# JingruiYu/FishBirdEyeVisualSLAM

Hardware: AMD Instinct MI355X
Metric: frames/s (extract+match+pose-opt), 1280x720+512x512 pair (higher is better)
Workload: dtype u8 (extract, Hamming) + f64 (pose optimisation); 1 GPU; configs[2]: 1280x720 front + 512x512 bird pair, HIP ORB extract + M3/M9 Hamming match + PoseOptimizationWithBird (~2k front + ~1k bird edges); nfeatures=2000, parallelism=replicas x1

## Files before the change

fishbirdeyevisualslam_amd/csrc/orb.hip:

```cpp
#include "fb_common.h"
#include "fb_fast_score.h"
#include "fb_primitives.h"

namespace {

constexpr int EDGE_THRESHOLD = 19;
constexpr int HALF_PATCH = 15;
constexpr int PATCH_SIZE = 31;
constexpr int BORDER = EDGE_THRESHOLD - 3;

constexpr int PATTERN_XY[1024] = {
#include "orb_pattern.inc"
};
constexpr int pattern_extreme(bool wantMax) {
  int m = PATTERN_XY[0];
  for (int i = 1; i < 1024; i++) m = wantMax ? (PATTERN_XY[i] > m ? PATTERN_XY[i] : m) : (PATTERN_XY[i] < m ? PATTERN_XY[i] : m);
  return m;
}
constexpr int PAT_BIAS = -pattern_extreme(false);
static_assert(PAT_BIAS >= 0 && pattern_extreme(true) + PAT_BIAS <= 255, "a pattern coordinate does not fit a biased byte");
struct PackedPattern { uint32_t test[256]; };
constexpr PackedPattern pack_pattern() {
  PackedPattern p{};
  for (int t = 0; t < 256; t++)
    for (int k = 0; k < 4; k++) p.test[t] |= (uint32_t)(PATTERN_XY[t * 4 + k] + PAT_BIAS) << (8 * k);
  return p;
}
__constant__ PackedPattern c_pattern = pack_pattern();

struct LevelInfo {
  int w, h, pitch;
  long long off;
  int nCols, nRows, wCell, hCell, cellBase;
  int N;
  long long candBase;
  int candCap;
  int slotCap;
  int outBase, outCap;
  int nIni;
  float hX;
  float scale;
  int patchSize;
  long long boff;
};

struct OrbK {
  int nlevels, iniTh, minTh, totalCells, outStride, capOut;
  int kpStride;
  int fastTileBytes, fastMaxOut, fastMaxPix;
  int fastTP;
  int dbg;
  unsigned long long *timers;
  int cellBase[FB_MAX_LEVELS + 1];
  int grpBase[FB_MAX_LEVELS + 1];
  int totalGroups;
  int descBase[FB_MAX_LEVELS + 1];
  int runBase[FB_MAX_LEVELS];
  int runCap[FB_MAX_LEVELS];
  long long pyrStride;
  long long blurStride;
  int blurStrips[FB_MAX_LEVELS + 1];
  long long candStride;
  int umax[16];
  LevelInfo L[FB_MAX_LEVELS];
};

struct ResizeTabs {
  const int *xofs;
  const short *ialpha;
  const int *yofs;
  const short *ibeta;
};

__device__ __forceinline__ int win_byte(uint32_t w0, uint32_t w1, uint32_t w2, uint32_t w3, int k) {
  const uint32_t lo = k & 8 ? w2 : w0, hi = k & 8 ? w3 : w1;
  const uint32_t w = k & 4 ? hi : lo;
  return (w >> (8 * (k & 3))) & 0xFF;
}

__global__ __launch_bounds__(256) void k_resize(const uint8_t *__restrict__ src0, long long srcImgStride, int sw,
                                                int sh, int spitch, uint8_t *__restrict__ dst0, long long dstImgStride,
                                                int dw, int dh, int dpitch, ResizeTabs tb) {
// ... 792 lines not shown
        const int r0 = min(tid * perj, J), r1 = min(r0 + perj, J);
        for (int r = r0; r < r1; r++) {
          const int p = order[r];
          for (int q = 0; q < 4; q++)
            if (ccnt[4 * p + q] > 0) {
              const int pos = totalKids - 1 - ci++;
              cpos[4 * p + q] = (unsigned short)pos;
              nxt[pos] = child_of(cur[p], q, ccnt[4 * p + q]);
            }
        }
        for (int p = a0; p < a1; p++)
          if (!split[p]) { npos[p] = (unsigned short)kp; nxt[kp++] = cur[p]; }
      }
    }
    const int Snew = totalKids + totalKeep;
    __syncthreads();
    for (int k0 = tid; k0 < n; k0 += NT * 4) {
      int pk[4];
      uint32_t ck[4];
#pragma unroll
      for (int u = 0; u < 4; u++) { const int kk = min(k0 + u * NT, n - 1); pk[u] = nof[kk]; ck[u] = cd[kk]; }
#pragma unroll
      for (int u = 0; u < 4; u++) {
        const int k = k0 + u * NT;
        if (k >= n) break;
        const int p = pk[u];
        if (split[p]) {
          const uint32_t c = ck[u];
          nof[k] = cpos[4 * p + quadrant(cur[p], (int)(c & 0xFFF) - BORDER, (int)((c >> 12) & 0xFFF) - BORDER)];
        } else nof[k] = npos[p];
      }
    }
    int myExp = 0;
    {
      const int pern = (Snew + NT - 1) / NT;
      const int n0 = min(tid * pern, Snew), n1 = min(n0 + pern, Snew);
      for (int p = n0; p < n1; p++) myExp += (p < totalKids && nxt[p].cnt > 1);
    }
    int nToExpand;
    fb::block_excl_scan<NT>(myExp, s_w, &nToExpand);
    if (tid == 0) s_nexp = nToExpand;
    __syncthreads();
    ONode *t = cur; cur = nxt; nxt = t;
    S = Snew;
    if (S >= N || S == prevSize) break;
    if (!finalPhase) {
      if (S + nToExpand * 3 > N) finalPhase = true;
    }
  }
  for (int p = tid; p < S; p += NT) best[p] = 0ull;
  __syncthreads();
  for (int k0 = tid; k0 < n; k0 += NT * 4) {
    int pk[4];
    uint32_t ck[4];
#pragma unroll
    for (int u = 0; u < 4; u++) { const int kk = min(k0 + u * NT, n - 1); pk[u] = nof[kk]; ck[u] = cd[kk]; }
#pragma unroll
    for (int u = 0; u < 4; u++) {
    const int k = k0 + u * NT;
    if (k >= n) break;
    const uint32_t c = ck[u];
    const int x = c & 0xFFF, y = (c >> 12) & 0xFFF, r = c >> 24;
    const int cellI = (y - EDGE_THRESHOLD) / Lv.hCell, cellJ = (x - EDGE_THRESHOLD) / Lv.wCell;
    const int dwid = min(Lv.wCell, Lv.w - 2 * EDGE_THRESHOLD - cellJ * Lv.wCell);
    const int inCell = (y - EDGE_THRESHOLD - cellI * Lv.hCell) * dwid + (x - EDGE_THRESHOLD - cellJ * Lv.wCell);
    const unsigned orderKey = (unsigned)(cellI * Lv.nCols + cellJ) * 4096u + (unsigned)inCell;
    const unsigned long long key = ((unsigned long long)r << 56) | ((unsigned long long)(0xFFFFFFFFu - orderKey) << 24) | (unsigned)k;
    atomicMax(&best[pk[u]], key);
    }
  }
  __syncthreads();
  for (int p = tid; p < S; p += NT) out[p] = cd[(unsigned)(best[p] & 0xFFFFFFull)];
  if (tid == 0) *outCount = S;
}

constexpr int BLUR_ROWS = 32;

__device__ __forceinline__ int reflect101(int i, int n) {
  if (i < 0) i = -i;
  if (i >= n) i = 2 * n - 2 - i;
  return i;
}

__global__ __launch_bounds__(256) void k_blur(OrbK K, const uint8_t *__restrict__ img0, long long imgStride, int pitch0,
                                              const uint8_t *__restrict__ pyr, uint8_t *__restrict__ blur) {
  const int b = blockIdx.y;
  const int strip = __builtin_amdgcn_readfirstlane(blockIdx.x * 4 + (threadIdx.x >> 6));
  const int lane = threadIdx.x & 63;
  if (strip >= K.blurStrips[K.nlevels]) return;
  int l = 0;
  while (strip >= K.blurStrips[l + 1]) l++;
  const LevelInfo &L = K.L[l];
  const int w = L.w, h = L.h;
  const int sidx = strip - K.blurStrips[l];
  const int nsx = (w + 255) >> 8;
  const int sy = sidx / nsx, sx = sidx - sy * nsx;
  const int x0 = sx * 256 + lane * 4;
  const int y0 = sy * BLUR_ROWS;
  if (x0 >= w) return;
  const uint8_t *img;
  int pitch;
  if (l == 0) { img = img0 + (long long)b * imgStride; pitch = pitch0; }
  else { img = pyr + (long long)b * K.pyrStride + L.off; pitch = L.pitch; }
  uint8_t *out = blur + (long long)b * K.blurStride + L.boff;
  const bool edge = x0 < 4 || x0 + 8 > w;
  const int base = edge ? max(min(x0 - 4, w - 12), 0) : x0 - 4;
  uint32_t m1[3] = {0, 0, 0}, m2[3] = {0, 0, 0};
  if (edge) {
#pragma unroll
    for (int i = 0; i < 12; i++) {
      const int c = reflect101(min(x0 - 4 + i, w + 2), w);
      const int sidx8 = min(max(c - base, 0), 11);
      const uint32_t lo = sidx8 < 8 ? (uint32_t)sidx8 : 0x0cu, hi = sidx8 < 8 ? 0x0cu : (uint32_t)(sidx8 - 8);
      m1[i >> 2] |= lo << (8 * (i & 3));
      m2[i >> 2] |= hi << (8 * (i & 3));
    }
  }
  const bool anyEdge = __ballot(edge) != 0ull;
  const uint32_t WA = 18u | (34u << 8) | (49u << 16) | (55u << 24), WB = 49u | (34u << 8) | (18u << 16);
  uint32_t pairs[6][4];
  uint32_t prevh[4] = {0u, 0u, 0u, 0u};
  constexpr int BLUR_PF = 4;
  uint32_t q[BLUR_PF][3];
  auto loadRow = [&](int r, uint32_t (&dst)[3]) {
    const int ys = reflect101(min(y0 + r - 3, h + 2), h);
    const uint8_t *row = img + (uint32_t)__mul24(ys, pitch);
    const uint32_t *pw = reinterpret_cast<const uint32_t *>(row + base);
    dst[0] = pw[0]; dst[1] = pw[1]; dst[2] = pw[2];
  };
#pragma unroll
  for (int r = 0; r < BLUR_PF; r++) loadRow(r, q[r]);
#pragma unroll
  for (int r = 0; r < BLUR_ROWS + 6; r++) {
    const int yo = y0 + r - 6;
    if (r >= 6 && yo >= h) break;
    uint32_t w0 = q[r % BLUR_PF][0], w1 = q[r % BLUR_PF][1], w2 = q[r % BLUR_PF][2];
    if (r + BLUR_PF < BLUR_ROWS + 6) loadRow(r + BLUR_PF, q[r % BLUR_PF]);
    if (anyEdge) {
      const uint32_t e0 = __builtin_amdgcn_perm(w1, w0, m1[0]) | __builtin_amdgcn_perm(w2, w2, m2[0]);
      const uint32_t e1 = __builtin_amdgcn_perm(w1, w0, m1[1]) | __builtin_amdgcn_perm(w2, w2, m2[1]);
      const uint32_t e2 = __builtin_amdgcn_perm(w1, w0, m1[2]) | __builtin_amdgcn_perm(w2, w2, m2[2]);
      if (edge) { w0 = e0; w1 = e1; w2 = e2; }
    }
    uint32_t hr[4];
    hr[0] = __builtin_amdgcn_udot4(__builtin_amdgcn_alignbyte(w2, w1, 1), WB, __builtin_amdgcn_udot4(__builtin_amdgcn_alignbyte(w1, w0, 1), WA, 0u, false), false);
    hr[1] = __builtin_amdgcn_udot4(__builtin_amdgcn_alignbyte(w2, w1, 2), WB, __builtin_amdgcn_udot4(__builtin_amdgcn_alignbyte(w1, w0, 2), WA, 0u, false), false);
    hr[2] = __builtin_amdgcn_udot4(__builtin_amdgcn_alignbyte(w2, w1, 3), WB, __builtin_amdgcn_udot4(__builtin_amdgcn_alignbyte(w1, w0, 3), WA, 0u, false), false);
    hr[3] = __builtin_amdgcn_udot4(w2, WB, __builtin_amdgcn_udot4(w1, WA, 0u, false), false);
    if (r >= 6) {
      typedef unsigned short u16x2b __attribute__((ext_vector_type(2)));
      const u16x2b W01 = {18, 34}, W23 = {49, 55}, W45 = {49, 34};
      uint32_t packed = 0;
#pragma unroll
      for (int k = 0; k < 4; k++) {
        uint32_t sum = (uint32_t)__mul24(18, (int)hr[k]) + (1u << 15);
        sum = __builtin_amdgcn_udot2(__builtin_bit_cast(u16x2b, pairs[(r + 1) % 6][k]), W01, sum, false);
        sum = __builtin_amdgcn_udot2(__builtin_bit_cast(u16x2b, pairs[(r + 3) % 6][k]), W23, sum, false);
        sum = __builtin_amdgcn_udot2(__builtin_bit_cast(u16x2b, pairs[(r + 5) % 6][k]), W45, sum, false);
        packed |= (uint32_t)min((int)(sum >> 16), 255) << (8 * k);
      }
      *reinterpret_cast<uint32_t *>(out + (uint32_t)(__mul24(yo, L.pitch) + x0)) = packed;
    }
#pragma unroll
    for (int k = 0; k < 4; k++) { pairs[r % 6][k] = prevh[k] | (hr[k] << 16); prevh[k] = hr[k]; }
  }
}

constexpr int DP_RAW_DW = 9, DP_RAW_ROWS = 31;
constexpr int DP_BL_DW = 10, DP_BL_ROWS = 37;

constexpr int DESC_WPB = 4;
constexpr int DESC_KPW = 2;

__global__ __launch_bounds__(64 * DESC_WPB) __attribute__((amdgpu_waves_per_eu(5, 5)))
void k_describe(OrbK K, const uint8_t *__restrict__ img0, long long imgStride,
                                                 int pitch0, const uint8_t *__restrict__ pyr,
                                                 const uint8_t *__restrict__ blur, const uint4 *__restrict__ angTab,
                                                 const uint32_t *__restrict__ lvlOut, const int *__restrict__ lvlCount,
                                                 fb_keypoint *__restrict__ kps, uint8_t *__restrict__ desc,
                                                 int32_t *__restrict__ nOut) {
  __shared__ __attribute__((aligned(16))) uint32_t rawp_all[DESC_WPB][DP_RAW_ROWS * DP_RAW_DW + 4];
  __shared__ __attribute__((aligned(16))) uint32_t blp_all[DESC_WPB][DP_BL_ROWS * DP_BL_DW + 2];
  const int b = blockIdx.y, lane = threadIdx.x & 63;
  const int wv = __builtin_amdgcn_readfirstlane(threadIdx.x >> 6);
  uint32_t *rawp = rawp_all[wv], *blp = blp_all[wv];
  const uint4 pq = reinterpret_cast<const uint4 *>(c_pattern.test)[lane];
  const uint4 angT = angTab[lane < 62 ? lane : 0];
  const int wg = (int)(blockIdx.x & 7) * (int)(gridDim.x >> 3) + (int)(blockIdx.x >> 3);
  int l = 0, runBase = K.runBase[0], runCap = K.runCap[0];
#pragma unroll
  for (int i = 1; i < FB_MAX_LEVELS; i++)
    if (i < K.nlevels && wg >= K.descBase[i]) { l = i; runBase = K.runBase[i]; runCap = K.runCap[i]; }
  const int slot = ((wg - K.descBase[l]) * DESC_WPB + wv) * DESC_KPW;
  const uint32_t *run = lvlOut + (long long)b * K.outStride + runBase;
  uint32_t rec[DESC_KPW];
#pragma unroll
  for (int j = 0; j < DESC_KPW; j++) rec[j] = run[min(slot + j, runCap - 1)];
  const int *cnts = lvlCount + b * K.nlevels;
  int below = 0, total = 0, mine = 0;
#pragma unroll
  for (int i = 0; i < FB_MAX_LEVELS; i++) {
    const int ci = cnts[i];
    const int c = i < K.nlevels ? ci : 0;
    total += c; below += i < l ? c : 0; mine = i == l ? c : mine;
  }
  const LevelInfo &Lv = K.L[l];
  const int lvPitch = Lv.pitch, lvPatch = Lv.patchSize;
  const long long lvOff = Lv.off, lvBoff = Lv.boff;
  const float lvScale = Lv.scale;
  const int nk = min(total, K.capOut);
  if (wg == 0 && threadIdx.x == 0) nOut[b] = nk;
  const int first = below + slot;
  const int nmine = min(DESC_KPW, min(mine - slot, nk - first));
  if (K.dbg == 11) { if ((int)(pq.x + pq.w) + (int)angT.x + (int)rec[0] + (int)rec[DESC_KPW - 1] + nmine + lvPitch + lvPatch + (int)lvOff + (int)lvBoff + (int)lvScale == 1234567) nOut[0] = 1; return; }
  if (nmine <= 0) return;
  const uint4 angW = make_uint4(angT.x & 0x0f0f0f0fu, angT.y & 0x0f0f0f0fu, angT.z & 0x0f0f0f0fu, angT.w & 0x0f0f0f0fu);
  const uint4 angK = make_uint4((angT.x >> 4) & 0x01010101u, (angT.y >> 4) & 0x01010101u, (angT.z >> 4) & 0x01010101u, (angT.w >> 4) & 0x01010101u);
  const uint8_t *lvImg = l == 0 ? img0 + (long long)b * imgStride : pyr + (long long)b * K.pyrStride + lvOff;
  const int rawPitch = l == 0 ? pitch0 : lvPitch;
  const uint8_t *lvBlur = blur + (long long)b * K.blurStride + lvBoff;
  const bool rawAligned = ((reinterpret_cast<uintptr_t>(lvImg) | (uintptr_t)rawPitch) & 3) == 0;
  constexpr int NB_IT = (DP_BL_ROWS + 5) / 6, NR_IT = (DP_RAW_ROWS + 6) / 7;
  const int rb0 = (lane * 205) >> 11, dwb = lane - rb0 * DP_BL_DW;
  const int rr0 = (lane * 57) >> 9, dwr = lane - rr0 * DP_RAW_DW;
  struct KP {
    int cx, cy, resp, pitch, bpitch, bxa, box, rxa, rox;
    const uint8_t *img, *bbase;
    bool rawAligned;
  };
  auto decode = [&](int j) {
    KP k;
    const uint32_t r = rec[j];
    k.cx = r & 0xFFF; k.cy = (r >> 12) & 0xFFF; k.resp = r >> 24;
    k.img = lvImg; k.pitch = rawPitch; k.bbase = lvBlur; k.bpitch = lvPitch; k.rawAligned = rawAligned;
    k.bxa = (k.cx - 18) & ~3; k.box = (k.cx - 18) - k.bxa;
    k.rxa = (k.cx - 15) & ~3;
    k.rox = k.rawAligned ? (k.cx - 15) - k.rxa : 0;
    return k;
  };
  uint32_t vb[DESC_KPW][NB_IT], vr[DESC_KPW][NR_IT];
  auto issue = [&](const KP &k, uint32_t (&vb)[NB_IT], uint32_t (&vr)[NR_IT]) {
    {
      uint32_t off = (uint32_t)(__mul24(k.cy - 18 + rb0, k.bpitch) + k.bxa + min(dwb, DP_BL_DW - 1) * 4);
// ... 27 lines not shown
      for (int i = lane; i < DP_RAW_ROWS * 31; i += 64) {
        const int yy = i / 31, xx = i - yy * 31;
        rb[yy * (DP_RAW_DW * 4) + xx] = k.img[(long long)(k.cy - 15 + yy) * k.pitch + k.cx - 15 + xx];
      }
    }
    __builtin_amdgcn_fence(__ATOMIC_RELEASE, "wavefront");
    __builtin_amdgcn_wave_barrier();
    __builtin_amdgcn_fence(__ATOMIC_ACQUIRE, "wavefront");
  };
  KP kpv[DESC_KPW];
#pragma unroll
  for (int j = 0; j < DESC_KPW; j++) {
    kpv[j] = decode(j);
    if (j < nmine) issue(kpv[j], vb[j], vr[j]);
  }
#pragma unroll
  for (int j = 0; j < DESC_KPW; j++) {
    if (j >= nmine) break;
    const KP &cur = kpv[j];
    stage(cur, vb[j], vr[j]);
    int m10 = 0, m01 = 0;
    if (lane < 62) {
      const int r = lane >> 1, half = lane & 1;
      const int sb = cur.rox + (half ? 15 : 0);
      const uint32_t *rowd = rawp + r * DP_RAW_DW + (sb >> 2);
      const uint32_t sh = (uint32_t)(sb & 3);
      const uint32_t d0 = rowd[0], d1 = rowd[1], d2 = rowd[2], d3 = rowd[3], d4 = rowd[4];
      const uint32_t q0 = __builtin_amdgcn_alignbyte(d1, d0, sh), q1 = __builtin_amdgcn_alignbyte(d2, d1, sh);
      const uint32_t q2 = __builtin_amdgcn_alignbyte(d3, d2, sh), q3 = __builtin_amdgcn_alignbyte(d4, d3, sh);
      const uint4 W = angW, Km = angK;
      const uint32_t a10 = __builtin_amdgcn_udot4(q0, W.x, __builtin_amdgcn_udot4(q1, W.y, __builtin_amdgcn_udot4(q2, W.z, __builtin_amdgcn_udot4(q3, W.w, 0u, false), false), false), false);
      const uint32_t rs = __builtin_amdgcn_udot4(q0, Km.x, __builtin_amdgcn_udot4(q1, Km.y, __builtin_amdgcn_udot4(q2, Km.z, __builtin_amdgcn_udot4(q3, Km.w, 0u, false), false), false), false);
      m10 = half ? (int)a10 : -(int)a10;
      m01 = __mul24(r - 15, (int)rs);
    }
    m10 = fb::wave_sum(m10);
    m01 = fb::wave_sum(m01);
    if (K.dbg == 12) { if (m10 + m01 == 12345678 && (int)(pq.x + pq.w) == 77777) nOut[0] = 1; continue; }
    const float angle = fb_fast_atan2((float)m01, (float)m10);
    const float factorPI = 0x1.1df46ap-6f;
    float sa, ca;
    fb_sincos_f(angle * factorPI, &sa, &ca);
    const float a = ca, bb = sa;
    const uint8_t *centre = reinterpret_cast<const uint8_t *>(blp) + 18 * (DP_BL_DW * 4) + cur.box + 18;
    int nib = 0;
#pragma unroll
    for (int t = 0; t < 4; t++) {
      const uint32_t p = t == 0 ? pq.x : t == 1 ? pq.y : t == 2 ? pq.z : pq.w;
      const float x0 = (float)(p & 0xFFu) - (float)PAT_BIAS, y0 = (float)((p >> 8) & 0xFFu) - (float)PAT_BIAS;
      const float x1 = (float)((p >> 16) & 0xFFu) - (float)PAT_BIAS, y1 = (float)(p >> 24) - (float)PAT_BIAS;
      const int t0 = centre[__mul24(fb_cvround(x0 * bb + y0 * a), DP_BL_DW * 4) + fb_cvround(x0 * a - y0 * bb)];
      const int t1 = centre[__mul24(fb_cvround(x1 * bb + y1 * a), DP_BL_DW * 4) + fb_cvround(x1 * a - y1 * bb)];
      nib |= (t0 < t1) << t;
    }
    const int hi = __shfl_down(nib, 1, 64);
    const int byteVal = nib | (hi << 4);
    const int b1 = __shfl_down(byteVal, 2, 64), b2 = __shfl_down(byteVal, 4, 64), b3 = __shfl_down(byteVal, 6, 64);
    const uint32_t dw = (uint32_t)byteVal | ((uint32_t)b1 << 8) | ((uint32_t)b2 << 16) | ((uint32_t)b3 << 24);
    const long long o = (long long)b * K.kpStride + first + j;
    if ((lane & 7) == 0) reinterpret_cast<uint32_t *>(desc + o * 32)[lane >> 3] = dw;
    if (lane == 0) {
      fb_keypoint kp;
      kp.x = (float)cur.cx;
      kp.y = (float)cur.cy;
      if (l != 0) { kp.x *= lvScale; kp.y *= lvScale; }
      kp.size = (float)lvPatch;
      kp.angle = angle;
      kp.response = (float)cur.resp;
      kp.octave = l;
      kps[o] = kp;
    }
    __builtin_amdgcn_fence(__ATOMIC_RELEASE, "wavefront");
    __builtin_amdgcn_wave_barrier();
  }
}

}

struct fb_orb {
  fb_orb_params p;
  fb_orb_tables t;
  hipStream_t sideStream = nullptr;
  hipEvent_t evFork = nullptr, evJoin = nullptr;
  ~fb_orb() {
    if (evFork) (void)hipEventDestroy(evFork);
    if (evJoin) (void)hipEventDestroy(evJoin);
    if (sideStream) (void)hipStreamDestroy(sideStream);
  }
  int kpStride = 0;
  int w = 0, h = 0, batchCap = 0;
  OrbK K;
  int maxNodes = 0;
  size_t octreeLds = 0;
  fb::DevBuf pyr, blur, cand, cellCand, cellCount, nodeOf, counts, lvlOut, tabs, angTab, timers;
  ResizeTabs rt[FB_MAX_LEVELS];
  bool mergeOK[FB_MAX_LEVELS] = {};
  bool rowsOK[FB_MAX_LEVELS] = {};
  const uint8_t *lastImg = nullptr;
  long long lastImgStride = 0;
  int lastPitch0 = 0;
  fb::DevBuf ownedImg;
};

namespace {

void make_tables(const fb_orb_params &p, fb_orb_tables &t) {
  memset(&t, 0, sizeof(t));
  const int nl = p.nlevels;
  t.scale_factor[0] = 1.0f;
  t.level_sigma2[0] = 1.0f;
  for (int i = 1; i < nl; i++) {
    t.scale_factor[i] = t.scale_factor[i - 1] * p.scale_factor;
    t.level_sigma2[i] = t.scale_factor[i] * t.scale_factor[i];
  }
  for (int i = 0; i < nl; i++) {
    t.inv_scale_factor[i] = 1.0f / t.scale_factor[i];
    t.inv_level_sigma2[i] = 1.0f / t.level_sigma2[i];
  }
  float factor = 1.0f / p.scale_factor;
  float nDesired = p.nfeatures * (1 - factor) / (1 - (float)pow((double)factor, (double)nl));
  int sum = 0;
  for (int l = 0; l < nl - 1; l++) {
    t.features_per_level[l] = fb_cvround(nDesired);
    sum += t.features_per_level[l];
    nDesired *= factor;
  }
  t.features_per_level[nl - 1] = std::max(p.nfeatures - sum, 0);
  int umax[HALF_PATCH + 2] = {0};
  int v, v0;
  const int vmax = fb_cvfloor(HALF_PATCH * sqrtf(2.f) / 2 + 1);
  const int vmin = fb_cvceil(HALF_PATCH * sqrtf(2.f) / 2);
  const double hp2 = HALF_PATCH * HALF_PATCH;
  for (v = 0; v <= vmax; ++v) umax[v] = fb_cvround_d(sqrt(hp2 - v * v));
  for (v = HALF_PATCH, v0 = 0; v >= vmin; --v) {
    while (umax[v0] == umax[v0 + 1]) ++v0;
    umax[v] = v0;
    ++v0;
  }
  for (int i = 0; i <= HALF_PATCH; i++) t.umax[i] = umax[i];
}

int capacity_of(const fb_orb_params &p) { return p.nfeatures + 8 * p.nlevels; }

int prepare(fb_orb *o, int w, int h, int batch) {
  if (o->w == w && o->h == h && batch <= o->batchCap) return FB_OK;
  const fb_orb_params &p = o->p;
  OrbK &K = o->K;
  memset(&K, 0, sizeof(K));
  K.nlevels = p.nlevels;
  K.iniTh = p.ini_th_fast;
  K.minTh = p.min_th_fast;
  K.capOut = capacity_of(p);
  K.kpStride = o->kpStride > 0 ? o->kpStride : K.capOut;
  for (int i = 0; i < 16; i++) K.umax[i] = o->t.umax[i];
  long long pyrOff = 0, candOff = 0, blurOff = 0;
  int cells = 0, outOff = 0, maxNodes = 0, strips = 0;
  std::vector<int> xofs, yofs;
  std::vector<short> ialpha, ibeta;
  std::vector<size_t> tabOff(p.nlevels * 4, 0);
  std::vector<uint8_t> tabBytes;
  auto append = [&](const void *src, size_t n) {
    size_t off = (tabBytes.size() + 15) & ~(size_t)15;
    tabBytes.resize(off + n);
    memcpy(tabBytes.data() + off, src, n);
    return off;
  };
  int pw = w, ph = h;
  for (int l = 0; l < p.nlevels; l++) {
    LevelInfo &L = K.L[l];
// ... 146 lines not shown
    o->rt[l].xofs = reinterpret_cast<const int *>(base + tabOff[l * 4 + 0]);
    o->rt[l].ialpha = reinterpret_cast<const short *>(base + tabOff[l * 4 + 1]);
    o->rt[l].yofs = reinterpret_cast<const int *>(base + tabOff[l * 4 + 2]);
    o->rt[l].ibeta = reinterpret_cast<const short *>(base + tabOff[l * 4 + 3]);
  }
  const size_t B = batch;
  {
    std::vector<uint32_t> tab(64 * 4, 0);
    for (int lane = 0; lane < 62; lane++) {
      const int v = (lane >> 1) - 15, half = lane & 1, dmax = K.umax[v < 0 ? -v : v];
      for (int j = 0; j < 16; j++) {
        const int au = half ? j : 15 - j;
        const bool inc = au <= dmax && (half || au != 0);
        if (!inc) continue;
        tab[lane * 4 + (j >> 2)] |= ((uint32_t)au | 0x10u) << (8 * (j & 3));
      }
    }
    FB_TRY(o->angTab.upload(tab.data(), tab.size() * 4));
  }
  FB_TRY(o->pyr.alloc(B * K.pyrStride + 256));
  FB_TRY(o->blur.alloc(B * K.blurStride + 256));
  FB_TRY(o->cand.alloc(B * K.candStride * 4 + 16));
  FB_TRY(o->cellCand.alloc(B * K.candStride * 4 + 16));
  FB_TRY(o->cellCount.alloc(B * (size_t)K.totalCells * 4 + 16));
  FB_TRY(o->nodeOf.alloc(B * K.candStride * 2 + 16));
  FB_TRY(o->counts.alloc(B * p.nlevels * 4 * 2 + FB_MAX_LEVELS * 4));
  FB_TRY(o->timers.alloc(FB_ORB_TIMER_WORDS * 8));
  FB_HIP(hipMemset(o->timers.p, 0, FB_ORB_TIMER_WORDS * 8));
  K.timers = o->timers.as<unsigned long long>();
  FB_TRY(o->lvlOut.alloc(B * K.outStride * 4 + 16));
  o->w = w; o->h = h; o->batchCap = batch;
  return FB_OK;
}

}

extern "C" {

int fb_orb_capacity(const fb_orb_params *params) {
  if (!params) return FB_ERR_ARG;
  return capacity_of(*params);
}

int fb_orb_set_output_stride(fb_orb *h, int kp_stride) {
  FB_ARG(h && (kp_stride == 0 || kp_stride >= capacity_of(h->p)));
  h->kpStride = kp_stride;
  h->K.kpStride = kp_stride > 0 ? kp_stride : capacity_of(h->p);
  return FB_OK;
}

int fb_orb_create(const fb_orb_params *params, fb_orb **out) {
  FB_ARG(params && out);
  FB_ARG(params->nlevels >= 1 && params->nlevels <= FB_MAX_LEVELS);
  FB_ARG(params->nfeatures >= 1 && params->nfeatures <= 60000);
  FB_ARG(params->scale_factor > 1.0f);
  FB_ARG(params->min_th_fast >= 1 && params->ini_th_fast >= params->min_th_fast && params->ini_th_fast <= 254);
  fb_orb *o = new fb_orb();
  o->p = *params;
  make_tables(o->p, o->t);
  *out = o;
  return FB_OK;
}

void fb_orb_destroy(fb_orb *h) { delete h; }

int fb_orb_get_tables(const fb_orb *h, fb_orb_tables *out) {
  FB_ARG(h && out);
  *out = h->t;
  return FB_OK;
}

int fb_orb_extract_batch_dev(fb_orb *o, const uint8_t *d_images, int batch, int width, int height, int stride,
                             size_t image_stride, fb_keypoint *d_keypoints, uint8_t *d_descriptors, int32_t *d_n,
                             void *stream) {
  FB_TRY(fb::check_device());
  FB_ARG(o && d_images && d_keypoints && d_descriptors && d_n);
  FB_ARG(batch >= 1 && width >= 2 * EDGE_THRESHOLD + 7 && height >= 2 * EDGE_THRESHOLD + 7 && stride >= width);
  FB_TRY(prepare(o, width, height, batch));
  hipStream_t s = fb::as_stream(stream);
  const OrbK &K = o->K;
  const int nl = K.nlevels;
  int *candCount = o->counts.as<int>();
  int *lvlCount = candCount + (size_t)o->batchCap * nl;
  FB_HIP(hipMemsetAsync(o->cellCount.p, 0, (size_t)batch * K.totalCells * 4, s));
  for (int l = 1; l < nl; l++) {
    const LevelInfo &D = K.L[l], &S = K.L[l - 1];
    const uint8_t *src = (l == 1) ? d_images : o->pyr.as<uint8_t>() + S.off;
    const long long sstr = (l == 1) ? (long long)image_stride : K.pyrStride;
    const int spitch = (l == 1) ? stride : S.pitch;
    dim3 blk(64, 4), grd((D.pitch / 4 + 63) / 64, (D.h + 3) / 4, batch);
    fb::ProfScope prof_(fb::P_RESIZE, s);
    const bool rows = o->rowsOK[l] && spitch >= 12 && ((reinterpret_cast<uintptr_t>(src) | (uintptr_t)spitch | (uintptr_t)sstr) & 3) == 0;
    if (rows && o->mergeOK[l]) {
      dim3 grdM((D.pitch / 4 + 63) / 64, (D.h + 4 * RM_ROWS - 1) / (4 * RM_ROWS), batch);
      k_resize_merge<<<grdM, blk, 0, s>>>(src, sstr, S.w, S.h, spitch, o->pyr.as<uint8_t>() + D.off, K.pyrStride, D.w, D.h, D.pitch, o->rt[l]);
    } else if (rows) {
      dim3 grdR((D.pitch / 4 + 63) / 64, (D.h + 4 * RESIZE_ROWS - 1) / (4 * RESIZE_ROWS), batch);
      k_resize_rows<<<grdR, blk, 0, s>>>(src, sstr, S.w, S.h, spitch, o->pyr.as<uint8_t>() + D.off, K.pyrStride, D.w, D.h, D.pitch, o->rt[l]);
    } else {
      k_resize<<<grd, blk, 0, s>>>(src, sstr, S.w, S.h, spitch, o->pyr.as<uint8_t>() + D.off, K.pyrStride, D.w, D.h, D.pitch, o->rt[l]);
    }
  }
  if (K.totalCells > 0) {
    fb::ProfScope prof_(K.fastTP == 44 ? fb::P_FAST : K.fastTP == 56 ? fb::P_FAST56 : fb::P_FAST72, s);
    const dim3 grdF((K.totalGroups + 7) / 8 * 8, batch);
    const size_t ldsF = (size_t)2 * K.fastTileBytes + 2 * K.fastMaxPix;
#define FAST_LAUNCH(TP_) { if (K.dbg == 20) k_fast<TP_, true><<<grdF, 64, ldsF, s>>>(K, d_images, (long long)image_stride, stride, o->pyr.as<uint8_t>(), o->cellCand.as<uint32_t>(), o->cellCount.as<int>()); \
                          else k_fast<TP_, false><<<grdF, 64, ldsF, s>>>(K, d_images, (long long)image_stride, stride, o->pyr.as<uint8_t>(), o->cellCand.as<uint32_t>(), o->cellCount.as<int>()); }
    if (K.fastTP == 44)
      FAST_LAUNCH(44)
    else if (K.fastTP == 56)
      FAST_LAUNCH(56)
    else
      FAST_LAUNCH(FAST_MAX_TILE)
#undef FAST_LAUNCH
  }
  static const int sideMin = [] {
    const char* e = getenv("FB_ORB_SIDE_MIN");
    return e ? atoi(e) : 64;
  }();
  const bool fork = batch >= sideMin && !(fb::g_prof_on && fb::g_prof_only < 0);
  hipStream_t sBlur = s;
  if (fork) {
    if (!o->sideStream) {
      FB_HIP(hipStreamCreateWithFlags(&o->sideStream, hipStreamNonBlocking));
      FB_HIP(hipEventCreateWithFlags(&o->evFork, hipEventDisableTiming));
      FB_HIP(hipEventCreateWithFlags(&o->evJoin, hipEventDisableTiming));
    }
    sBlur = o->sideStream;
    FB_HIP(hipEventRecord(o->evFork, s));
    FB_HIP(hipStreamWaitEvent(sBlur, o->evFork, 0));
  }
#ifndef FB_ORB_ABLATE_BLUR
  {
    fb::ProfScope prof_(fb::P_BLUR, sBlur);
    k_blur<<<dim3((K.blurStrips[nl] + 3) / 4, batch), 256, 0, sBlur>>>(K, d_images, (long long)image_stride, stride, o->pyr.as<uint8_t>(),
                                                                        o->blur.as<uint8_t>());
  }
#endif
  if (fork) FB_HIP(hipEventRecord(o->evJoin, sBlur));
  static const int octWideMax = getenv("FB_OCT_WIDE_MAX") ? atoi(getenv("FB_OCT_WIDE_MAX")) : 512;
  const bool octWide = nl * batch <= octWideMax;
  FB_HIP(hipFuncSetAttribute(octWide ? reinterpret_cast<const void *>(k_octree<1024>) : reinterpret_cast<const void *>(k_octree<256>), hipFuncAttributeMaxDynamicSharedMemorySize, (int)o->octreeLds));
  {
  fb::ProfScope prof_(fb::P_OCTREE, s);
  if (octWide)
    k_octree<1024><<<dim3(batch, nl), 1024, o->octreeLds, s>>>(K, o->cellCand.as<uint32_t>(), o->cellCount.as<int>(), o->cand.as<uint32_t>(), candCount, o->nodeOf.as<uint16_t>(),
                                                          o->lvlOut.as<uint32_t>(), lvlCount, o->maxNodes);
  else
    k_octree<256><<<dim3(batch, nl), 256, o->octreeLds, s>>>(K, o->cellCand.as<uint32_t>(), o->cellCount.as<int>(), o->cand.as<uint32_t>(), candCount, o->nodeOf.as<uint16_t>(),
                                                         o->lvlOut.as<uint32_t>(), lvlCount, o->maxNodes);
  }
  if (fork) FB_HIP(hipStreamWaitEvent(s, o->evJoin, 0));
  {
  fb::ProfScope prof_(fb::P_DESCRIBE, s);
  k_describe<<<dim3((K.descBase[nl] + 7) / 8 * 8, batch), 64 * DESC_WPB, 0, s>>>(K, d_images, (long long)image_stride, stride, o->pyr.as<uint8_t>(),
                                                   o->blur.as<uint8_t>(), o->angTab.as<uint4>(), o->lvlOut.as<uint32_t>(), lvlCount, d_keypoints,
                                                   d_descriptors, d_n);
  }
  FB_HIP(hipGetLastError());
  o->lastImg = d_images;
  o->lastImgStride = (long long)image_stride;
  o->lastPitch0 = stride;
  return FB_OK;
}

int fb_orb_extract(fb_orb *o, const uint8_t *image, int width, int height, int stride, fb_keypoint *keypoints,
                   uint8_t *descriptors, int32_t *n_out) {
  FB_TRY(fb::check_device());
  FB_ARG(o && n_out);
  if (!image || width <= 0 || height <= 0) return FB_OK;
  FB_ARG(keypoints && descriptors && stride >= width);
  const int cap = capacity_of(o->p);
  const size_t imgBytes = (size_t)stride * height, kpBytes = (size_t)cap * sizeof(fb_keypoint), dBytes = (size_t)cap * 32;
  const size_t oN = 0, oK = 256, oD = oK + ((kpBytes + 255) & ~(size_t)255), oC = oD + ((dBytes + 255) & ~(size_t)255), outBytes = oC + 256;
  const size_t imgArea = fb::Stager::up256(imgBytes);
  uint8_t *pin = static_cast<uint8_t *>(fb::pinned_scratch(imgArea + outBytes));
  if (!pin) return FB_ERR_HIP;
  fb::DevBuf dout;
  FB_TRY(dout.alloc(outBytes));
  if (o->ownedImg.bytes < imgBytes || !o->ownedImg.p) FB_TRY(o->ownedImg.alloc(imgBytes));
  memcpy(pin, image, imgBytes);
  struct SyncOnError {
    bool armed = true;
    ~SyncOnError() { if (armed) { (void)hipStreamSynchronize(nullptr); (void)hipGetLastError(); } }
  } guard;
  FB_HIP(hipMemcpyAsync(o->ownedImg.p, pin, imgBytes, hipMemcpyHostToDevice, nullptr));
  uint8_t *dbase = dout.as<uint8_t>();
  const int keepStride = o->kpStride;
  if (keepStride) FB_TRY(fb_orb_set_output_stride(o, 0));
  const int rc = fb_orb_extract_batch_dev(o, o->ownedImg.as<uint8_t>(), 1, width, height, stride, imgBytes, reinterpret_cast<fb_keypoint *>(dbase + oK),
                                          dbase + oD, reinterpret_cast<int32_t *>(dbase + oN), nullptr);
  if (keepStride) (void)fb_orb_set_output_stride(o, keepStride);
  FB_TRY(rc);
  uint8_t *pout = pin + imgArea;
  FB_HIP(hipMemcpyAsync(pout, dbase, oC, hipMemcpyDeviceToHost, nullptr));
  FB_HIP(hipMemcpyAsync(pout + oC, o->counts.as<int>() + (size_t)o->batchCap * o->p.nlevels, (size_t)o->p.nlevels * 4, hipMemcpyDeviceToHost, nullptr));
  FB_HIP(hipStreamSynchronize(nullptr));
  guard.armed = false;
  memcpy(n_out, pout + oN, 4);
  {
    const int *lc = reinterpret_cast<const int *>(pout + oC);
    int total = 0;
    for (int l = 0; l < o->p.nlevels; l++) total += lc[l];
    if (total > cap) {
      fb::set_error("keypoint capacity exceeded: the quadtree kept %d key points, fb_orb_capacity() is %d", total, cap);
      return FB_ERR_CAPACITY;
    }
  }
  memcpy(keypoints, pout + oK, (size_t)*n_out * sizeof(fb_keypoint));
  memcpy(descriptors, pout + oD, (size_t)*n_out * 32);
  return FB_OK;
}

int fb_orb_debug_timers(fb_orb *o, uint64_t *dst16) {
  FB_TRY(fb::check_device());
  FB_ARG(o && dst16 && o->timers.p);
  FB_HIP(hipDeviceSynchronize());
  FB_HIP(hipMemcpy(dst16, o->timers.p, 16 * 8, hipMemcpyDeviceToHost));
  FB_HIP(hipMemset(o->timers.p, 0, 16 * 8));
  return FB_OK;
}

// ... 51 lines not shown
```

Baseline: 75860 frames/s.

## Split blur by pyramid level, interleave with resize, and cut blur ALU ops

```diff
diff --git a/fishbirdeyevisualslam_amd/csrc/orb.hip b/fishbirdeyevisualslam_amd/csrc/orb.hip
--- a/fishbirdeyevisualslam_amd/csrc/orb.hip
+++ b/fishbirdeyevisualslam_amd/csrc/orb.hip
@@ -1,3 +1,5 @@
+#include <climits>
+
 #include "fb_common.h"
 #include "fb_fast_score.h"
 #include "fb_primitives.h"
@@ -956,13 +958,13 @@
   return i;
 }
 
-__global__ __launch_bounds__(256) void k_blur(OrbK K, const uint8_t *__restrict__ img0, long long imgStride, int pitch0,
+__global__ __launch_bounds__(256) void k_blur(OrbK K, int l0, int l1, const uint8_t *__restrict__ img0, long long imgStride, int pitch0,
                                               const uint8_t *__restrict__ pyr, uint8_t *__restrict__ blur) {
   const int b = blockIdx.y;
-  const int strip = __builtin_amdgcn_readfirstlane(blockIdx.x * 4 + (threadIdx.x >> 6));
+  const int strip = __builtin_amdgcn_readfirstlane(K.blurStrips[l0] + blockIdx.x * 4 + (threadIdx.x >> 6));
   const int lane = threadIdx.x & 63;
-  if (strip >= K.blurStrips[K.nlevels]) return;
-  int l = 0;
+  if (strip >= K.blurStrips[l1]) return;
+  int l = l0;
   while (strip >= K.blurStrips[l + 1]) l++;
   const LevelInfo &L = K.L[l];
   const int w = L.w, h = L.h;
@@ -991,9 +993,14 @@
     }
   }
   const bool anyEdge = __ballot(edge) != 0ull;
-  const uint32_t WA = 18u | (34u << 8) | (49u << 16) | (55u << 24), WB = 49u | (34u << 8) | (18u << 16);
+  constexpr uint32_t W0A = (18u << 8) | (34u << 16) | (49u << 24), W0B = 55u | (49u << 8) | (34u << 16) | (18u << 24);
+  constexpr uint32_t W1A = (18u << 16) | (34u << 24), W1B = 49u | (55u << 8) | (49u << 16) | (34u << 24), W1C = 18u;
+  constexpr uint32_t W2A = 18u << 24, W2B = 34u | (49u << 8) | (55u << 16) | (49u << 24), W2C = 34u | (18u << 8);
+  constexpr uint32_t W3B = 18u | (34u << 8) | (49u << 16) | (55u << 24), W3C = 49u | (34u << 8) | (18u << 16);
   uint32_t pairs[6][4];
   uint32_t prevh[4] = {0u, 0u, 0u, 0u};
+  uint32_t rnd = 1u << 15;
+  asm volatile("" : "+s"(rnd));
   constexpr int BLUR_PF = 4;
   uint32_t q[BLUR_PF][3];
   auto loadRow = [&](int r, uint32_t (&dst)[3]) {
@@ -1017,22 +1024,25 @@
       if (edge) { w0 = e0; w1 = e1; w2 = e2; }
     }
     uint32_t hr[4];
-    hr[0] = __builtin_amdgcn_udot4(__builtin_amdgcn_alignbyte(w2, w1, 1), WB, __builtin_amdgcn_udot4(__builtin_amdgcn_alignbyte(w1, w0, 1), WA, 0u, false), false);
-    hr[1] = __builtin_amdgcn_udot4(__builtin_amdgcn_alignbyte(w2, w1, 2), WB, __builtin_amdgcn_udot4(__builtin_amdgcn_alignbyte(w1, w0, 2), WA, 0u, false), false);
-    hr[2] = __builtin_amdgcn_udot4(__builtin_amdgcn_alignbyte(w2, w1, 3), WB, __builtin_amdgcn_udot4(__builtin_amdgcn_alignbyte(w1, w0, 3), WA, 0u, false), false);
-    hr[3] = __builtin_amdgcn_udot4(w2, WB, __builtin_amdgcn_udot4(w1, WA, 0u, false), false);
+    hr[0] = __builtin_amdgcn_udot4(w1, W0B, __builtin_amdgcn_udot4(w0, W0A, 0u, false), false);
+    hr[1] = __builtin_amdgcn_udot4(w2, W1C, __builtin_amdgcn_udot4(w1, W1B, __builtin_amdgcn_udot4(w0, W1A, 0u, false), false), false);
+    hr[2] = __builtin_amdgcn_udot4(w2, W2C, __builtin_amdgcn_udot4(w1, W2B, __builtin_amdgcn_udot4(w0, W2A, 0u, false), false), false);
+    hr[3] = __builtin_amdgcn_udot4(w2, W3C, __builtin_amdgcn_udot4(w1, W3B, 0u, false), false);
     if (r >= 6) {
       typedef unsigned short u16x2b __attribute__((ext_vector_type(2)));
       const u16x2b W01 = {18, 34}, W23 = {49, 55}, W45 = {49, 34};
-      uint32_t packed = 0;
+      uint32_t sum[4];
 #pragma unroll
       for (int k = 0; k < 4; k++) {
-        uint32_t sum = (uint32_t)__mul24(18, (int)hr[k]) + (1u << 15);
-        sum = __builtin_amdgcn_udot2(__builtin_bit_cast(u16x2b, pairs[(r + 1) % 6][k]), W01, sum, false);
-        sum = __builtin_amdgcn_udot2(__builtin_bit_cast(u16x2b, pairs[(r + 3) % 6][k]), W23, sum, false);
-        sum = __builtin_amdgcn_udot2(__builtin_bit_cast(u16x2b, pairs[(r + 5) % 6][k]), W45, sum, false);
-        packed |= (uint32_t)min((int)(sum >> 16), 255) << (8 * k);
-      }
+        sum[k] = (uint32_t)__mul24(18, (int)hr[k]) + rnd;
+        sum[k] = __builtin_amdgcn_udot2(__builtin_bit_cast(u16x2b, pairs[(r + 1) % 6][k]), W01, sum[k], false);
+        sum[k] = __builtin_amdgcn_udot2(__builtin_bit_cast(u16x2b, pairs[(r + 3) % 6][k]), W23, sum[k], false);
+        sum[k] = __builtin_amdgcn_udot2(__builtin_bit_cast(u16x2b, pairs[(r + 5) % 6][k]), W45, sum[k], false);
+      }
+      const u16x2b C255 = {255, 255};
+      const u16x2b h01 = __builtin_elementwise_min(__builtin_bit_cast(u16x2b, __builtin_amdgcn_perm(sum[1], sum[0], 0x07060302u)), C255);
+      const u16x2b h23 = __builtin_elementwise_min(__builtin_bit_cast(u16x2b, __builtin_amdgcn_perm(sum[3], sum[2], 0x07060302u)), C255);
+      const uint32_t packed = __builtin_amdgcn_perm(__builtin_bit_cast(uint32_t, h23), __builtin_bit_cast(uint32_t, h01), 0x06040200u);
       *reinterpret_cast<uint32_t *>(out + (uint32_t)(__mul24(yo, L.pitch) + x0)) = packed;
     }
 #pragma unroll
@@ -1226,9 +1236,12 @@
   fb_orb_tables t;
   hipStream_t sideStream = nullptr;
   hipEvent_t evFork = nullptr, evJoin = nullptr;
+  hipEvent_t evLevel[FB_MAX_LEVELS] = {};
   ~fb_orb() {
     if (evFork) (void)hipEventDestroy(evFork);
     if (evJoin) (void)hipEventDestroy(evJoin);
+    for (hipEvent_t e : evLevel)
+      if (e) (void)hipEventDestroy(e);
     if (sideStream) (void)hipStreamDestroy(sideStream);
   }
   int kpStride = 0;
@@ -1541,13 +1554,58 @@
   const int nl = K.nlevels;
   int *candCount = o->counts.as<int>();
   int *lvlCount = candCount + (size_t)o->batchCap * nl;
+  static const int sideMin = [] {
+    const char* e = getenv("FB_ORB_SIDE_MIN");
+    return e ? atoi(e) : INT_MAX;
+  }();
+  static const unsigned blurCutsEnv = [] {
+    const char* e = getenv("FB_ORB_BLUR_CUTS");
+    return e ? (unsigned)strtoul(e, nullptr, 0) : 0u;
+  }();
+  const bool profAll = fb::g_prof_on && fb::g_prof_only < 0;
+  const bool fork = batch >= sideMin && !profAll;
+  const unsigned blurCuts = profAll ? 0u : blurCutsEnv;
+  auto blurLevels = [&](int l0, int l1, hipStream_t st) {
+#ifndef FB_ORB_ABLATE_BLUR
+    const int strips = K.blurStrips[l1] - K.blurStrips[l0];
+    if (strips <= 0) return;
+    fb::ProfScope prof_(fb::P_BLUR, st);
+    k_blur<<<dim3((strips + 3) / 4, batch), 256, 0, st>>>(K, l0, l1, d_images, (long long)image_stride, stride, o->pyr.as<uint8_t>(), o->blur.as<uint8_t>());
+#endif
+  };
+  hipStream_t sBlur = s;
+  int blurFrom = 0;
+  auto blurBehind = [&](int l) -> int {
+    if (l + 1 < nl && !((blurCuts >> (l + 1)) & 1u)) return FB_OK;
+    if (fork && l > 0) {
+      FB_HIP(hipEventRecord(o->evLevel[l], s));
+      FB_HIP(hipStreamWaitEvent(sBlur, o->evLevel[l], 0));
+    }
+    blurLevels(blurFrom, l + 1, sBlur);
+    blurFrom = l + 1;
+    return FB_OK;
+  };
+  if (fork) {
+    if (!o->sideStream) {
+      if (!o->evFork) FB_HIP(hipEventCreateWithFlags(&o->evFork, hipEventDisableTiming));
+      if (!o->evJoin) FB_HIP(hipEventCreateWithFlags(&o->evJoin, hipEventDisableTiming));
+      for (int l = 1; l < FB_MAX_LEVELS; l++)
+        if (!o->evLevel[l]) FB_HIP(hipEventCreateWithFlags(&o->evLevel[l], hipEventDisableTiming));
+      FB_HIP(hipStreamCreateWithFlags(&o->sideStream, hipStreamNonBlocking));
+    }
+    sBlur = o->sideStream;
+    FB_HIP(hipEventRecord(o->evFork, s));
+    FB_HIP(hipStreamWaitEvent(sBlur, o->evFork, 0));
+  }
   FB_HIP(hipMemsetAsync(o->cellCount.p, 0, (size_t)batch * K.totalCells * 4, s));
+  FB_TRY(blurBehind(0));
   for (int l = 1; l < nl; l++) {
     const LevelInfo &D = K.L[l], &S = K.L[l - 1];
     const uint8_t *src = (l == 1) ? d_images : o->pyr.as<uint8_t>() + S.off;
     const long long sstr = (l == 1) ? (long long)image_stride : K.pyrStride;
     const int spitch = (l == 1) ? stride : S.pitch;
     dim3 blk(64, 4), grd((D.pitch / 4 + 63) / 64, (D.h + 3) / 4, batch);
+    {
     fb::ProfScope prof_(fb::P_RESIZE, s);
     const bool rows = o->rowsOK[l] && spitch >= 12 && ((reinterpret_cast<uintptr_t>(src) | (uintptr_t)spitch | (uintptr_t)sstr) & 3) == 0;
     if (rows && o->mergeOK[l]) {
@@ -1559,7 +1617,10 @@
     } else {
       k_resize<<<grd, blk, 0, s>>>(src, sstr, S.w, S.h, spitch, o->pyr.as<uint8_t>() + D.off, K.pyrStride, D.w, D.h, D.pitch, o->rt[l]);
     }
-  }
+    }
+    FB_TRY(blurBehind(l));
+  }
+  if (fork) FB_HIP(hipEventRecord(o->evJoin, sBlur));
   if (K.totalCells > 0) {
     fb::ProfScope prof_(K.fastTP == 44 ? fb::P_FAST : K.fastTP == 56 ? fb::P_FAST56 : fb::P_FAST72, s);
     const dim3 grdF((K.totalGroups + 7) / 8 * 8, batch);
@@ -1574,30 +1635,6 @@
       FAST_LAUNCH(FAST_MAX_TILE)
 #undef FAST_LAUNCH
   }
-  static const int sideMin = [] {
-    const char* e = getenv("FB_ORB_SIDE_MIN");
-    return e ? atoi(e) : 64;
-  }();
-  const bool fork = batch >= sideMin && !(fb::g_prof_on && fb::g_prof_only < 0);
-  hipStream_t sBlur = s;
-  if (fork) {
-    if (!o->sideStream) {
-      FB_HIP(hipStreamCreateWithFlags(&o->sideStream, hipStreamNonBlocking));
-      FB_HIP(hipEventCreateWithFlags(&o->evFork, hipEventDisableTiming));
-      FB_HIP(hipEventCreateWithFlags(&o->evJoin, hipEventDisableTiming));
-    }
-    sBlur = o->sideStream;
-    FB_HIP(hipEventRecord(o->evFork, s));
-    FB_HIP(hipStreamWaitEvent(sBlur, o->evFork, 0));
-  }
-#ifndef FB_ORB_ABLATE_BLUR
-  {
-    fb::ProfScope prof_(fb::P_BLUR, sBlur);
-    k_blur<<<dim3((K.blurStrips[nl] + 3) / 4, batch), 256, 0, sBlur>>>(K, d_images, (long long)image_stride, stride, o->pyr.as<uint8_t>(),
-                                                                        o->blur.as<uint8_t>());
-  }
-#endif
-  if (fork) FB_HIP(hipEventRecord(o->evJoin, sBlur));
   static const int octWideMax = getenv("FB_OCT_WIDE_MAX") ? atoi(getenv("FB_OCT_WIDE_MAX")) : 512;
   const bool octWide = nl * batch <= octWideMax;
   FB_HIP(hipFuncSetAttribute(octWide ? reinterpret_cast<const void *>(k_octree<1024>) : reinterpret_cast<const void *>(k_octree<256>), hipFuncAttributeMaxDynamicSharedMemorySize, (int)o->octreeLds));
```

After: 81260 frames/s, median of 6. +7.1%, better.
